# hitmaxiang/pytorch-openpose

Hardware: AMD Instinct MI355X
Metric: frames/sec (body+PAF grouping) at 368x656 (higher is better)
Workload: dtype f32

## Files before the change

### include/opose.h

```cpp
#ifndef OPOSE_H
#define OPOSE_H

#include <stddef.h>
#include <stdint.h>

#ifdef __cplusplus
extern "C" {
#endif

typedef struct opose_ctx opose_t;

typedef enum opose_status {
    OPOSE_OK = 0,
    OPOSE_E_ARG = -1,
    OPOSE_E_SHAPE = -2,
    OPOSE_E_HIP = -3,
    OPOSE_E_WEIGHTS = -4,
    OPOSE_E_CAPACITY = -5,
    OPOSE_E_ASSEMBLY = -6,
    OPOSE_E_TIMEOUT = -7,
} opose_status;

enum { OPOSE_NET_BODY = 0, OPOSE_NET_HAND = 1 };

// ... 124 lines not shown

int opose_profile_enable(opose_t* h, int enable);
int opose_profile_reset(opose_t* h);
int opose_profile_read(opose_t* h, char* buf, size_t len);

int opose_debug_conv(opose_t* h, const float* x, const float* w, const float* b, int N, int Cin, int H, int W,
                     int Cout, int ks, int pad, int relu, int mt, int pt, int splits, float* out);
int opose_debug_conv_time(opose_t* h, int N, int Cin, int H, int W, int Cout, int ks, int ngroups,
                          int mt, int pt, int splits, int ablate, int reps, float* ms);
int opose_debug_conv_x6(opose_t* h, const float* x, const float* w, const float* b, int N, int Cin, int H,
                        int W, int Cout, int ks, int pad, int relu, int mt, int pt, int splits, int out_x6,
                        float* out);
int opose_debug_conv_segs(opose_t* h, int nseg, const int* geom, const float* const* x, int nw,
                          const float* const* w, const float* const* b, int Cin, int Cout, int ks, int relu,
                          int family, int pool, int in_padded, int out_kind, int out_total, int dup, int net,
                          int lvl, int pair, float* const* out, float* const* out_dup, int* ran,
                          int64_t* clobbered);
int opose_debug_chain(opose_t* h, int nseg, const int* geom, const float* const* x, int nw,
                      const float* const* w1, const float* const* b1, const float* const* w2,
                      const float* const* b2, int m1, int cout2, int relu2, int in_padded, int out_x6,
                      float* const* out);
int opose_debug_conv1(opose_t* h, int stage, int nseg, const int* geom, const float* const* x, const float* w,
                      const float* b, int f32, float* const* out);
int opose_debug_conv_x6_time(opose_t* h, int N, int Cin, int H, int W, int Cout, int ks, int ngroups,
                             int mt, int pt, int splits, int reps, float* ms);
int opose_debug_preprocess(opose_t* h, const uint8_t* bgr, int H, int W, double scale, int pad_value,
                           float* out, int* HpWp);
int opose_debug_preprocess_groups(opose_t* h, int n_groups, const uint8_t* const* bgr, const int* N,
                                  const int* H, const int* W, double scale, int pad_value,
                                  float* const* out, int* HpWp);
int opose_debug_heat(opose_t* h, const float* maps, int hl, int wl, int pad_down, int pad_right, int H, int W,
                     double* heat_avg, float* paf_mid);
int opose_debug_hand_label(opose_t* h, const double* maps, int NP, int H, int W, double thre, int32_t* labels,
                           double* sums);
int opose_debug_batch_preprocess(opose_t* h, const uint8_t* bgr, int N, int H, int W, int64_t row_stride,
                                 int64_t frame_stride, double boxsize, double scale, float* out, int* HpWp);
int opose_debug_batch_heat(opose_t* h, const float* maps, int N, int hl, int wl, int nh, int nw, int H, int W,
                           float* heat, float* mid);
int opose_debug_blur5_nms(opose_t* h, const float* heat, int NP, int H, int W, double thre, int cap, int32_t* cnt,
                          int32_t* list, double* score);
int opose_debug_batch_hand_label(opose_t* h, const float* heat, int NP, int H, int W, double thre, double* blurred,
                                 int32_t* labels, double* sums);
int opose_debug_peaks_finalize(opose_t* h, const int32_t* cnt, const int32_t* list, const double* score, int N,
                               int H, int W, void* records, int32_t* peak_pos, int32_t* part_cnt);
int opose_debug_paf_score(opose_t* h, int fast, int n_scales, const float* const* maps, const int* hl, const int* wl,
                          const int* ga, const int* gb, const int32_t* peak_pos, const int32_t* part_cnt, int N,
// ... 18 lines not shown
```

### pytorch-openpose_amd/csrc/conv_win.hip

```cpp
#include <algorithm>
#include <stdexcept>

#include "common.h"
#include "kernels.h"
#include "x6_loop.h"

namespace opose {

template <int MT, int PT, int KS, int WMAX, int NST>
__global__ __launch_bounds__(64 * x6_waves(MT, PT), 1) void conv_win_x6(X6Args a) {
    constexpr int TAPS = KS * KS, PAD = KS / 2;
    constexpr int NW = x6_waves(MT, PT), NWM = NW == 8 ? MT / 64 : 2, NWP = NW / NWM;
    constexpr int WM = MT / NWM, WP = PT / NWP;
    constexpr int TM = WM / 16, TN = WP / 16;
    constexpr int A_U = 12 * MT;
    constexpr int A_PW = A_U / 64 / NW;
    constexpr int WBUF = 3 * WMAX;
    static_assert(A_U % (64 * NW) == 0 && A_PW == 3 && WMAX % 64 == 0 && TAPS >= 9, "conv_win_x6 tile");
    static_assert(NST == 2 || NST == 3, "conv_win_x6 stages");
    constexpr int WOFF = NST * A_U;
    static_assert(TM * TN >= 3, "block 4 hosts the offset steps");

    __shared__ __attribute__((aligned(16))) uint4 lds[NST * A_U + 2 * WBUF];
    __shared__ float s_bias[MT];
// ... 24 lines not shown
        const int n = p / HW, y = (p - n * HW) / W;
        return 3 + n * (H + 3) + y;
    };
    const int p_last = min(p0 + PT, npix) - 1;
    const int R0 = prow(p0), R1 = prow(p_last);
    const int ws = (R0 - PAD) * P;
    const int L = (R1 - R0 + 2 * PAD + 1) * P + PAD;
    const int NQ = (L + 63) >> 6;
    const uint32_t plane0 = G.in_l.o0 - 3u * (uint32_t)P - 3u;
    const int cin_g = a.cin_g;

    auto dma_win = [&](int g) __attribute__((always_inline)) {
        const uint32_t src = (plane0 + (uint32_t)g * G.in_l.gs + (uint32_t)ws) * 16u;
        uint4* dst = lds + WOFF + (g & 1) * WBUF;
        for (int i = wave; i < 3 * NQ; i += NW) {
            const int pc = i / NQ, j = i - pc * NQ;
            const __amdgpu_buffer_rsrc_t rsrc = __builtin_amdgcn_make_buffer_rsrc(
                (void*)(G.in + (size_t)pc * G.in_ps), (short)0, (int)G.in_ps, 0x00020000);
            __builtin_amdgcn_raw_ptr_buffer_load_lds(rsrc, (lds_ptr_t)(dst + pc * WMAX + 64 * j), 16,
                                                     src + (uint32_t)(64 * j + lane) * 16u, 0, 0, 0);
        }
    };
    const uint32_t lane16 = (uint32_t)lane * 16u;
    auto dma_a_unit = [&](int c, int buf, int u) __attribute__((always_inline)) {
        const int unit0 = (wave * A_PW + u) * 64;
        const int pg = unit0 / MT, m = unit0 - pg * MT;
        x6_dma_weights_unit(x6_weights_rsrc(G.wt, a.Mpad, c), (lds_units_t)(lds + buf * A_U), unit0, lane16,
                            (uint32_t)(pg * a.Mpad + m0 + m) * 16u);
    };
    auto dma_a = [&](int c, int buf) __attribute__((always_inline)) {
#pragma unroll
        for (int u = 0; u < A_PW; ++u) dma_a_unit(c, buf, u);
    };

    const int gi = lane >> 4;
    uint32_t bbase[TN];
#pragma unroll
    for (int j = 0; j < TN; ++j) {
        const int p = min(p0 + wp0 + 16 * j + (lane & 15), npix - 1);
        const int n = p / HW, r = p - n * HW, y = r / W, x = r - y * W;
        const int wpos = (3 + n * (H + 3) + y) * P + 3 + x - ws;
        bbase[j] = (uint32_t)(uintptr_t)(lds_ptr_t)(lds + WOFF + wpos);
    }
    int pg_g = (4 * c_begin + gi) / TAPS, pg_t = (4 * c_begin + gi) % TAPS;
    int s_dy = 0, s_dx = 0;
    uint32_t off_n = 0;
    constexpr int OFF_STEPS = 3;
    auto off_step = [&](int k) __attribute__((always_inline)) {
        if (k == 0) {
            s_dy = pg_t / KS;
            s_dx = pg_t - s_dy * KS - PAD;
            s_dy -= PAD;
        } else if (k == 1) {
            off_n = (uint32_t)((min(pg_g, cin_g - 1) & 1) * WBUF * 16 + (s_dy * P + s_dx) * 16);
        } else {
            const int w = pg_t + 4 >= TAPS ? 1 : 0;
            pg_t = pg_t + 4 - w * TAPS;
            pg_g += w;
        }
    };
    auto off_all = [&]() __attribute__((always_inline)) {
#pragma unroll
        for (int k = 0; k < OFF_STEPS; ++k) off_step(k);
    };

    X6Frags<MT, TM, TN> f;
    f.zero();
    constexpr int NB = f.NB, TMN = f.TMN;
    const int a16 = (lane >> 4) * MT + wm0 + (lane & 15);
    auto la = [&](int buf) __attribute__((always_inline)) {
        return (uint32_t)(uintptr_t)(lds_ptr_t)(lds + buf * A_U + a16);
    };

    const int g_first = (4 * c_begin) / TAPS;
    dma_win(g_first);
    if (g_first + 1 < cin_g) dma_win(g_first + 1);
#pragma unroll
    for (int st = 0; st < NST; ++st) dma_a(min(c_begin + st, c_end - 1), st);
    asm volatile("s_waitcnt vmcnt(0)" ::: "memory");
    __syncthreads();
    X6BWin<TN, WMAX> bcur, bnxt;
    {
        off_all();
#pragma unroll
        for (int j = 0; j < TN; ++j) bnxt.a[j] = bbase[j] + off_n;
        off_all();
        f.rd_group(0, la(0), bnxt);
        f.rd_group(1, la(0), bnxt);
    }
    int end_g = g_first;
    int end_c = (g_first * TAPS + TAPS - 1) / 4;
    int buf = 0;
    for (int c = c_begin; c < c_end; ++c) {
        const int nbuf = buf + 1 == NST ? 0 : buf + 1;
        const uint32_t a_cur = la(buf), a_nxt = la(nbuf);
        const int c2 = min(c + NST, c_end - 1);
#pragma unroll
        for (int j = 0; j < TN; ++j) bcur.a[j] = bnxt.a[j];
#pragma unroll
        for (int j = 0; j < TN; ++j) bnxt.a[j] = bbase[j] + off_n;
        f.head(a_cur, bcur);
        f.template barrier<NST == 3 ? A_PW : 0>();
        if (c == end_c) {
            if (end_g + 2 < cin_g) dma_win(end_g + 2);
            ++end_g;
            end_c = (end_g * TAPS + TAPS - 1) / 4;
        }
        __builtin_amdgcn_sched_barrier(0);
#pragma unroll
        for (int q = 0; q < NB; ++q) {
            f.mf(3, q);
            constexpr int N3 = TMN + 1;
#pragma unroll
            for (int o = q * N3 / NB; o < (q + 1) * N3 / NB; ++o) {
                if (o < TMN) f.rd(0, o, a_nxt, bnxt);
                else dma_a_unit(c2, buf, 0);
            }
            __builtin_amdgcn_sched_barrier(0);
        }
#pragma unroll
        for (int q = 0; q < NB; ++q) {
            f.mf(4, q);
            constexpr int N4 = A_PW - 2;
#pragma unroll
            for (int o = q * N4 / NB; o < (q + 1) * N4 / NB; ++o) dma_a_unit(c2, buf, 1 + o);
            if (q < OFF_STEPS) off_step(q);
            __builtin_amdgcn_sched_barrier(0);
        }
#pragma unroll
        for (int q = 0; q < NB; ++q) {
            f.mf(5, q);
            constexpr int N5 = TMN + 1;
#pragma unroll
            for (int o = q * N5 / NB; o < (q + 1) * N5 / NB; ++o) {
                if (o < TMN) f.rd(1, o, a_nxt, bnxt);
                else dma_a_unit(c2, buf, A_PW - 1);
            }
            __builtin_amdgcn_sched_barrier(0);
        }
        buf = nbuf;
    }
    asm volatile("s_waitcnt vmcnt(0) lgkmcnt(0)" ::: "memory");
    f.fence_all();

    if (!un.whole) {
        const __amdgpu_buffer_rsrc_t srs = slab_rsrc(a.partial);
        const uint32_t sbase = (uint32_t)uid * (uint32_t)(MT * PT * 4);
#pragma unroll
        for (int j = 0; j < TN; ++j) {
            const int pl = wp0 + j * 16 + (lane & 15);
#pragma unroll
            for (int i = 0; i < TM; ++i) {
                const int q = (wm0 + i * 16) / 4 + (lane >> 4);
                store_slab_quad(srs, sbase + (uint32_t)(q * PT + pl) * 16u, f.acc[i][j]);
            }
        }
        continue;
    }
    const X6Out out = x6_out(G);
// ... 73 lines not shown
```

### pytorch-openpose_amd/csrc/conv_x6.hip

```cpp
#include <algorithm>
#include <cstdlib>
#include <stdexcept>

#include "common.h"
#include "kernels.h"
#include "x6_loop.h"

namespace opose {

template <int MT, int PT, bool SMALL, int KS>
__global__ __launch_bounds__(64 * x6_waves(MT, PT), 1) void conv_x6(X6Args a) {
    const int ks = KS ? KS : a.ks;
    const int taps = ks * ks;
    constexpr int NW = x6_waves(MT, PT), NWM = NW == 8 ? MT / 64 : 2, NWP = NW / NWM;
    constexpr int WM = MT / NWM, WP = PT / NWP;
    constexpr int TM = WM / 16, TN = WP / 16;
    constexpr int PJ = PT / 64;
    constexpr int A_U = 12 * MT, B_U = 12 * PT;
    constexpr int A_PW = A_U / 64 / NW;
    constexpr int WPJ = NW / PJ;
    constexpr int B_PW = 12 / WPJ;
    static_assert(NW % PJ == 0 && 12 % WPJ == 0 && A_U % (64 * NW) == 0, "x6 tile");

    constexpr int STAGE_U = A_U + B_U;
    __shared__ __attribute__((aligned(16))) uint4 lds[2 * STAGE_U];
// ... 150 lines not shown
            auto mf = [&](int t, int q) __attribute__((always_inline)) {
                const int i = q / TN, j = q % TN;
                acc[i][j] = mfma_x6(fa[kPieceA[t]][i], fb[kPieceB[t]][j], acc[i][j]);
            };
            auto fence_all = [&]() __attribute__((always_inline)) {
#pragma unroll
                for (int pc = 0; pc < 3; ++pc) {
#pragma unroll
                    for (int i = 0; i < TM; ++i) asm volatile("" : "+v"(fa[pc][i]));
#pragma unroll
                    for (int j = 0; j < TN; ++j) asm volatile("" : "+v"(fb[pc][j]));
                }
            };
            dma_a(c_begin, 0);
            dma_b(c_begin, 0);
            asm volatile("s_waitcnt vmcnt(0)" ::: "memory");
            __syncthreads();
            {
                const uint32_t a0 = la(0), b0 = lb(0);
#pragma unroll
                for (int r = 0; r < TMN; ++r) rd(0, r, a0, b0);
#pragma unroll
                for (int r = 0; r < TMN; ++r) rd(1, r, a0, b0);
                const int cn = min(c_begin + 1, c_end - 1);
                dma_a(cn, 1);
                dma_b(cn, 1);
            }
            for (int c = c_begin; c < c_end; ++c) {
                const int buf = (c - c_begin) & 1;
                const uint32_t a_cur = la(buf), b_cur = lb(buf);
                const uint32_t a_nxt = la(buf ^ 1), b_nxt = lb(buf ^ 1);
                const int c2 = min(c + 2, c_end - 1);
                const BPrep bp2 = b_prep(c2);
                asm volatile("s_waitcnt lgkmcnt(%0)" ::"i"(TMN > 15 ? 15 : TMN) : "memory");
                fence_all();
                __builtin_amdgcn_sched_barrier(0);
#pragma unroll
                for (int q = 0; q < NB; ++q) {
                    mf(0, q);
#pragma unroll
                    for (int r = q * TMN / NB; r < (q + 1) * TMN / NB; ++r) rd(2, r, a_cur, b_cur);
                    __builtin_amdgcn_sched_barrier(0);
                }
                asm volatile("s_waitcnt lgkmcnt(%0)" ::"i"(TMN > 15 ? 15 : TMN) : "memory");
                fence_all();
                __builtin_amdgcn_sched_barrier(0);
#pragma unroll
                for (int q = 0; q < NB; ++q) {
                    mf(1, q);
                    __builtin_amdgcn_sched_barrier(0);
                }
                asm volatile("s_waitcnt lgkmcnt(0)" ::: "memory");
                fence_all();
                __builtin_amdgcn_sched_barrier(0);
#pragma unroll
                for (int q = 0; q < NB; ++q) {
                    mf(2, q);
                    __builtin_amdgcn_sched_barrier(0);
                }
                asm volatile("s_waitcnt vmcnt(0)" ::: "memory");
                __syncthreads();
                __builtin_amdgcn_sched_barrier(0);
                constexpr int D3 = NDA / 3, D4 = 2 * NDA / 3;
                auto dma_op = [&](int d) __attribute__((always_inline)) {
                    if (d < A_PW) dma_a_unit(c2, buf, d);
                    else dma_b_unit(c2, bp2, buf, d - A_PW);
                };
#pragma unroll
                for (int q = 0; q < NB; ++q) {
                    mf(3, q);
                    constexpr int N3 = TMN + D3;
#pragma unroll
                    for (int o = q * N3 / NB; o < (q + 1) * N3 / NB; ++o) {
                        if (o < TMN) rd(0, o, a_nxt, b_nxt);
                        else dma_op(o - TMN);
                    }
                    __builtin_amdgcn_sched_barrier(0);
                }
#pragma unroll
                for (int q = 0; q < NB; ++q) {
                    mf(4, q);
                    constexpr int N4 = D4 - D3;
#pragma unroll
                    for (int o = q * N4 / NB; o < (q + 1) * N4 / NB; ++o) dma_op(D3 + o);
                    __builtin_amdgcn_sched_barrier(0);
                }
#pragma unroll
                for (int q = 0; q < NB; ++q) {
                    mf(5, q);
                    constexpr int N5 = TMN + NDA - D4;
#pragma unroll
                    for (int o = q * N5 / NB; o < (q + 1) * N5 / NB; ++o) {
                        if (o < TMN) rd(1, o, a_nxt, b_nxt);
                        else dma_op(D4 + o - TMN);
                    }
                    __builtin_amdgcn_sched_barrier(0);
                }
            }
            asm volatile("s_waitcnt lgkmcnt(0)" ::: "memory");
            fence_all();
        }

        const bool whole = un.whole;
        const X6Out out = x6_out(G);
        const int cout8 = out.cout8;
#pragma unroll
        for (int j = 0; j < TN; ++j) {
            const int pl = wp0 + j * 16 + (lane & 15);
            const int p = p0 + pl;
            auto quad_row = [&](int i) __attribute__((always_inline)) { return wm0 + i * 16 + 4 * (lane >> 4); };
            if (!whole) {
                const __amdgpu_buffer_rsrc_t srs = slab_rsrc(a.partial);
                const uint32_t sbase = (uint32_t)uid * (uint32_t)(MT * PT * 4);
#pragma unroll
                for (int i = 0; i < TM; ++i)
                    store_slab_quad(srs, sbase + (uint32_t)((quad_row(i) / 4) * PT + pl) * 16u, acc[i][j]);
                continue;
            }
            if (a.pool) {
                const int q = p >> 2;
                const int n = q / HWo;
// ... 698 lines not shown
```

### pytorch-openpose_amd/csrc/engine_debug.cpp

```cpp
#include "engine.h"

using namespace opose;

int opose_debug_conv(opose_t* h, const float* x, const float* w, const float* b, int N, int Cin, int H, int W,
                     int Cout, int ks, int pad, int relu, int mt, int pt, int splits, float* out) {
    if (!h || !x || !w || !b || !out || ks > 15 || pad > 7) return OPOSE_E_ARG;
    OPOSE_TRY(h, {
        enter_main(h);
        Spec s{"debug", Cin, Cout, ks, pad};
        upload_conv(h, 0, "__debug__", {&s}, {w}, {b}, 3, false);
        DevConv* c = h->convs[0]["__debug__"].get();
        DevBuf xin, yout;
        const size_t nx = (size_t)N * Cin * H * W, ny = (size_t)N * Cout * H * W;
        float* xd = xin.ensure<float>(nx, h->stream);
        float* yd = yout.ensure<float>(ny, h->stream);
        OPOSE_HIP_CHECK(hipMemcpyAsync(xd, x, nx * 4, hipMemcpyHostToDevice, h->stream));
        ConvArgs a{};
        a.N = N; a.H = H; a.W = W; a.Cin = Cin; a.ks = ks; a.pad = pad;
        a.K = c->K; a.Kpad = c->Kpad; a.Mpad = c->Mpad; a.npix = N * H * W;
        a.tap_major = c->tap_major ? 1 : 0;
        ConvGroup& G = a.g[0];
        G.in = xd; G.in_cstride = Cin; G.in_coff = 0; G.wt = c->wt; G.bias = c->bias;
        G.out = yd; G.out_cstride = Cout; G.out_coff = 0; G.out2 = nullptr; G.cout = Cout; G.relu = relu;
        a.g[1] = a.g[0];
// ... 109 lines not shown
        const uint32_t ips = (uint32_t)((size_t)N * cg * HW * 16), ops = (uint32_t)((size_t)N * og * HW * 16);
        float* xd = xin.ensure<float>(nx, h->stream);
        uint8_t* x6 = xx.ensure<uint8_t>((size_t)ips * 3, h->stream);
        uint8_t* y6 = yx.ensure<uint8_t>((size_t)ops * 3, h->stream);
        float* yd = yout.ensure<float>(ny, h->stream);
        OPOSE_HIP_CHECK(hipMemcpyAsync(xd, x, nx * 4, hipMemcpyHostToDevice, h->stream));
        launch_to_x6(xd, Cin, 0, Cin, N, HW, x6, cg, 0, ips, h->stream);
        X6Args a{};
        a.ks = ks; a.pad = pad;
        a.cin_g = cg; a.small = c->small6 ? 1 : 0; a.nK = c->nK6; a.Mpad = c->Mpad;
        X6Group& G = a.g[0];
        G.N = N; G.H = H; G.W = W; G.npix = N * HW;
        G.in = x6; G.in_ps = ips; G.in_l = x6act(x6, cg, 0, N, H, W).l;
        G.wt = c->wx6; G.bias = c->bias; G.cout = Cout; G.relu = relu; G.out2 = nullptr;
        if (out_x6) { G.out = y6; G.out_ps = ops; G.out_l = x6act(y6, og, 0, N, H, W).l; G.out_f32 = 0; }
        else { G.out = yd; G.out_c = Cout; G.out_off = 0; G.out_f32 = 1; }
        a.ngroups = 1;
        const TileChoice t = debug_x6_plan(h, a, mt, pt, splits);
        launch_conv_x6(a, t.mt, t.pt, h->stream);
        if (out_x6) launch_from_x6(y6, og, 0, ops, Cout, N, HW, yd, Cout, 0, h->stream);
        OPOSE_HIP_CHECK(hipMemcpyAsync(out, yd, ny * 4, hipMemcpyDeviceToHost, h->stream));
        OPOSE_HIP_CHECK(hipStreamSynchronize(h->stream));
        h->convs[0].erase("__debug__");
    });
    return OPOSE_OK;
}

struct DebugConvs {
    opose_ctx* h;
    int net;
    std::vector<std::string> keys;
    DevConv* add(const std::string& key, const Spec& s, const float* w, const float* b, int lvl, bool pair) {
        upload_conv(h, net, key, {&s}, {w}, {b}, lvl, pair);
        keys.push_back(key);
        return h->convs[net][key].get();
    }
    ~DebugConvs() {
        for (const std::string& k : keys) h->convs[net].erase(k);
    }
};

constexpr int kDebugFill = 0xa5;

static int64_t clobbered_units(const uint16_t* hy, const XAct& a, int og, int N, int H, int W) {
    const size_t units = a.ps / 16;
    std::vector<uint8_t> written(units, 0);
// ... 846 lines not shown
```

### pytorch-openpose_amd/csrc/engine_net.cpp

```cpp
#include "engine.h"

namespace opose {

static const NetTable& net_table(opose_ctx* h, int net) {
    if (!h->loaded[net]) throw std::runtime_error(std::string(net_desc(net).what) + " weights not loaded");
    return h->table[net];
}

static void record_gate(opose_ctx* h) {
    if (!h->gate_ev) return;
    OPOSE_HIP_CHECK(hipEventRecord(h->gate_ev, h->stream));
    h->gate_done = true;
}

static const char* conv_class(int ks) { return ks == 7 ? "conv7x7" : (ks == 3 ? "conv3x3" : "conv1x1"); }

static void run_conv(opose_ctx* h, DevConv* c0, DevConv* c1, int N, int H, int W, Act in0, Act out0, Act in1,
                     Act out1, bool relu0, bool relu1, Act dup = {nullptr, 0, 0}) {
    ConvArgs a{};
    const int ng = c1 ? 2 : 1;
    a.N = N;
    a.H = H;
    a.W = W;
    a.Cin = c0->cin;
// ... 118 lines not shown
static XAct frame_view(const XAct& a, int n, int H, int W) {
    XAct v = a;
    if (!a.p) return v;
    if (a.f32) v.p = static_cast<float*>(a.p) + (size_t)n * a.c * H * W;
    else v.l.o0 = a.l.o0 + (uint32_t)n * a.l.fs;
    return v;
}

static std::string layer_names(const std::vector<ConvSeg>& segs) {
    std::string nm = segs[0].c->name;
    for (size_t g = 1; g < segs.size(); ++g)
        if (segs[g].c != segs[0].c && nm.find(segs[g].c->name) == std::string::npos) nm += "|" + segs[g].c->name;
    return "layer/" + nm;
}

static void launch_segs(opose_ctx* h, const std::vector<ConvSeg>& segs, int family, bool pool) {
    const bool win = family == kKernelWin, wino = family == kKernelWino;
    DevConv* c0 = segs[0].c;
    X6Args a{};
    const int ng = (int)segs.size();
    a.ks = c0->ks;
    a.pad = c0->pad;
    a.cin_g = c0->cin_g;
    a.small = c0->small6 ? 1 : 0;
    a.nK = wino ? c0->nKw : win ? c0->nK6p : c0->nK6;
    a.Mpad = c0->Mpad;
    a.pool = pool ? 1 : 0;
    a.ngroups = ng;
    double flops = 0;
    long npix_all = 0;
    for (int g = 0; g < ng; ++g) {
        const ConvSeg& sg = segs[g];
        DevConv* c = sg.c;
        if (c->ks != c0->ks || c->cin_g != c0->cin_g || c->Mpad != c0->Mpad || c->nK6 != c0->nK6 || c->nK6p != c0->nK6p)
            throw std::invalid_argument("conv segments of different shapes");
        if (pool && (sg.dup.p || sg.out.f32)) throw std::invalid_argument("pooled conv: single X6 output only");
        X6Group& G = a.g[g];
        G.in = static_cast<const uint8_t*>(sg.in.p);
        G.in_ps = sg.in.ps;
        G.in_l = sg.in.l;
        G.wt = wino ? c->wwino : win ? c->wx6p : c->wx6;
        G.bias = c->bias;
        G.out = sg.out.p;
        G.out_ps = sg.out.ps;
        G.out_l = sg.out.l;
        G.out_c = sg.out.c;
        G.out_off = sg.out.off;
// ... 538 lines not shown
```

### pytorch-openpose_amd/csrc/engine_plan.cpp

```cpp
#include "engine.h"

namespace opose {

TileChoice choose_tile(int Mpad, const std::vector<int>& gpix, int nK, bool x6, bool dp_only, double* cost_out) {
    long npix_all = 0;
    for (int n : gpix) npix_all += n;
    static const int cfg[6][3] = {{128, 128, 2}, {128, 256, 1}, {256, 128, 1},
                                  {128, 64, 3},  {64, 128, 3},  {64, 64, 4}};
    static const int occ6[6] = {1, 1, 1, 2, 2, 3};
    static const double ovh6_big[6] = {1.5, 1.0, 0.96, 1.1, 1.1, 1.2};
    static const double ovh6_small[6] = {1.0, 1.0, 0.96, 1.1, 1.1, 1.6};
    const double* ovh6 = npix_all <= 16384 ? ovh6_small : ovh6_big;
    const double rate = x6 ? 0.4 : 1.0;
    static const double ovh[6] = {1.0, 0.95, 0.93, 1.02, 1.02, 1.06};
    TileChoice best{64, 64, 1};
    double best_cost = 1e300;
    for (int c = 0; c < 6; ++c) {
        const int mt = cfg[c][0], pt = cfg[c][1], occ = x6 ? occ6[c] : cfg[c][2];
        if (Mpad % mt) continue;
        long tiles = 0;
        for (int n : gpix) tiles += (long)(Mpad / mt) * ((n + pt - 1) / pt);
        const double unit = (mt / 64.0) * (pt / 64.0) * (x6 ? ovh6[c] : ovh[c]) * rate;
        const long per_cu = (tiles + 255) / 256;
        const double floor1 = occ >= 2 ? 1.6 : 1.0;
// ... 149 lines not shown
                          : 0;
    const std::string key = std::to_string(win) + "/" + std::to_string(nK) + "/" + std::to_string(c->Mpad) + "/" +
                            std::to_string(npix) + "/" + std::to_string(mult) + "/" + std::to_string(bpix);
    auto it = h->slab_cache.find(key);
    if (it != h->slab_cache.end()) return it->second;
    static const int cand[] = {1, 2, 3, 4, 5, 6, 7, 8, 10, 12, 14, 16, 20, 24, 28, 32, 40, 48, 64};
    int best = 1;
    double best_cost = 1e300;
    for (int S : cand) {
        if (S > std::max(1, smax)) break;
        double cost = pick_tile(std::vector<ColGroup>(mult, ColGroup{npix, S}), win, nK, c->Mpad).cost;
        if (bpix) cost += pick_tile(std::vector<ColGroup>(mult, ColGroup{bpix, S}), win, nK, c->Mpad, false, false).cost;
        if (cost < best_cost * 0.97) {
            best_cost = cost;
            best = S;
        }
    }
    h->slab_cache[key] = best;
    return best;
}

static int seg_kernel_direct(const opose_ctx* h, const ConvSeg& sg, bool pool) {
    const DevConv* c = sg.c;
    if (!h->win7 || pool || !c->wx6p || !sg.in.padded || (c->ks != 3 && c->ks != 7)) return kKernelX6;
    const long lpix = (long)sg.N * (sg.Hl ? sg.Hl : sg.H) * sg.W;
    if (c->net == OPOSE_NET_BODY && lpix < 4096) return kKernelX6;
    if (c->net == OPOSE_NET_HAND && c->ks == 3 && c->lvl == 3 && c->Mpad > 128) return kKernelX6;
    if (sg.N == 1) return conv_win_fits_rows(sg.W, c->ks) ? kKernelWin : kKernelX6;
    if (conv_win_fits(sg.N, sg.H, sg.W, c->ks)) return kKernelWin;
    if (c->ks == 7 && h->split_frames && conv_win_fits_rows(sg.W, c->ks)) return kKernelWinFrames;
    return kKernelX6;
}

int seg_kernel(opose_ctx* h, const ConvSeg& sg, bool pool) {
    if (h->force_kernel >= 0) return h->force_kernel;
    const int k = seg_kernel_direct(h, sg, pool);
    const DevConv* c = sg.c;
    if (k == kKernelWin && h->wino && c->ks == 3 && c->wwino &&
        slab_count(h, c, true, sg.N, sg.Hl ? sg.Hl : sg.H, sg.W, pool) == 1 &&
        wino_tpf(sg.N, sg.Hl ? sg.Hl : sg.H, sg.W) >= 0)
        return kKernelWino;
    return k;
}

ConvPlan plan_launch(opose_ctx* h, const std::vector<ConvSeg>& segs, bool win, bool pool, int nK, int Mpad) {
    std::string key = (win ? "w" : "x") + std::to_string(pool) + "/" + std::to_string(nK) + "/" + std::to_string(Mpad);
    for (const ConvSeg& s : segs)
// ... 39 lines not shown
```

### pytorch-openpose_amd/csrc/engine_weights.cpp

```cpp
#include "engine.h"

namespace opose {

static DevConv* find_conv(opose_ctx* h, int net, const std::string& name) {
    auto it = h->convs[net].find(name);
    if (it == h->convs[net].end()) throw std::runtime_error("missing layer " + name);
    return it->second.get();
}

void upload_conv(opose_ctx* h, int net, const std::string& key, const std::vector<const Spec*>& parts,
                 const std::vector<const float*>& w, const std::vector<const float*>& b, int lvl, bool pair,
                 const std::vector<int>& cmap) {
    auto dc = std::make_unique<DevConv>();
    const Spec& s0 = *parts[0];
    dc->name = key;
    dc->net = net;
    dc->lvl = lvl;
    dc->pair = pair;
    dc->cin = s0.cin;
    dc->ks = s0.ks;
    dc->pad = s0.pad;
    dc->K = s0.cin * s0.ks * s0.ks;
    dc->tap_major = s0.cin >= 32;
    const int cin_pad = round_up(s0.cin, 32);
// ... 18 lines not shown
    std::vector<int> ktab(dc->Kpad, 0);
    for (int k = 0; k < dc->K; ++k) {
        int c = k / (dc->ks * dc->ks), r = k % (dc->ks * dc->ks);
        ktab[k] = (c << 8) | ((r / dc->ks) << 4) | (r % dc->ks);
    }
    {
        const int cin_phys = cmap.empty() ? s0.cin : cmap.back() + 1;
        const int taps = s0.ks * s0.ks;
        std::vector<float> wp((size_t)cout * cin_phys * taps, 0.f);
        int mm = 0;
        for (size_t i = 0; i < parts.size(); ++i)
            for (int m = 0; m < parts[i]->cout; ++m, ++mm)
                for (int c = 0; c < s0.cin; ++c) {
                    const int pc = cmap.empty() ? c : cmap[c];
                    for (int t = 0; t < taps; ++t)
                        wp[((size_t)mm * cin_phys + pc) * taps + t] = w[i][((size_t)m * s0.cin + c) * taps + t];
                }
        std::vector<uint16_t> wx;
        x6_pack_weights(wp.data(), cout, cin_phys, s0.ks, dc->Mpad, &dc->nK6, wx);
        dc->cin_g = (cin_phys + 7) / 8;
        dc->small6 = dc->cin_g == 1;
        OPOSE_HIP_CHECK(hipMalloc(&dc->wx6, wx.size() * 2));
        OPOSE_HIP_CHECK(hipMemcpy(dc->wx6, wx.data(), wx.size() * 2, hipMemcpyHostToDevice));
        if ((s0.ks == 7 || s0.ks == 3) && dc->Mpad % 128 == 0 && cin_phys > 8) {
            x6_pack_weights_pairs(wp.data(), cout, cin_phys, s0.ks, dc->Mpad, &dc->nK6p, wx);
            OPOSE_HIP_CHECK(hipMalloc(&dc->wx6p, wx.size() * 2));
            OPOSE_HIP_CHECK(hipMemcpy(dc->wx6p, wx.data(), wx.size() * 2, hipMemcpyHostToDevice));
        }
        if (s0.ks == 3 && dc->Mpad % 128 == 0 && cin_phys > 8) {
            x6_pack_weights_wino(wp.data(), cout, cin_phys, dc->Mpad, &dc->nKw, wx);
            OPOSE_HIP_CHECK(hipMalloc(&dc->wwino, wx.size() * 2));
            OPOSE_HIP_CHECK(hipMemcpy(dc->wwino, wx.data(), wx.size() * 2, hipMemcpyHostToDevice));
        }
    }
    OPOSE_HIP_CHECK(hipMalloc(&dc->wt, wt.size() * 4));
    OPOSE_HIP_CHECK(hipMalloc(&dc->bias, bias.size() * 4));
    OPOSE_HIP_CHECK(hipMalloc(&dc->ktab, ktab.size() * 4));
    g_alloc_epoch.fetch_add(1);
    OPOSE_HIP_CHECK(hipMemcpy(dc->wt, wt.data(), wt.size() * 4, hipMemcpyHostToDevice));
    OPOSE_HIP_CHECK(hipMemcpy(dc->bias, bias.data(), bias.size() * 4, hipMemcpyHostToDevice));
    OPOSE_HIP_CHECK(hipMemcpy(dc->ktab, ktab.data(), ktab.size() * 4, hipMemcpyHostToDevice));
    h->convs[net][key] = std::move(dc);
}

}

using namespace opose;
// ... 50 lines not shown
```

### pytorch-openpose_amd/csrc/x6.h

```cpp
#pragma once
#include <hip/hip_runtime.h>

#include "common.h"

namespace opose {

typedef float f32x4 __attribute__((ext_vector_type(4)));
typedef __bf16 bf16x8 __attribute__((ext_vector_type(8)));
typedef int i32x4 __attribute__((ext_vector_type(4)));
typedef __attribute__((address_space(3))) void* lds_ptr_t;
typedef __attribute__((address_space(3))) uint4* lds_units_t;

namespace x6 {

constexpr int x6_waves(int mt, int pt) { return mt * pt >= 32768 ? 8 : 4; }

__device__ __forceinline__ uint32_t bf16_rne(float x) {
    uint32_t u = __float_as_uint(x);
    u += 0x7fffu + ((u >> 16) & 1u);
    return u >> 16;
}

__device__ __forceinline__ void split3(float x, uint32_t& h0, uint32_t& h1, uint32_t& h2) {
    h0 = bf16_rne(x);
    const float r = x - __uint_as_float(h0 << 16);
    h1 = bf16_rne(r);
    const float r2 = r - __uint_as_float(h1 << 16);
    h2 = bf16_rne(r2);
}

__device__ __forceinline__ float join3(uint32_t h0, uint32_t h1, uint32_t h2) {
    return (__uint_as_float(h0 << 16) + __uint_as_float(h1 << 16)) + __uint_as_float(h2 << 16);
}

__device__ __forceinline__ void pack_pieces4(const float (&v)[4], uint2 (&w)[3]) {
    uint32_t h[3][4];
#pragma unroll
    for (int t = 0; t < 4; ++t) split3(v[t], h[0][t], h[1][t], h[2][t]);
#pragma unroll
    for (int pc = 0; pc < 3; ++pc) {
        w[pc].x = h[pc][0] | (h[pc][1] << 16);
        w[pc].y = h[pc][2] | (h[pc][3] << 16);
    }
}
__device__ __forceinline__ void pack_pieces8(const float (&v)[8], uint4 (&w)[3]) {
    uint32_t h[3][8];
#pragma unroll
    for (int t = 0; t < 8; ++t) split3(v[t], h[0][t], h[1][t], h[2][t]);
#pragma unroll
    for (int pc = 0; pc < 3; ++pc) {
        w[pc].x = h[pc][0] | (h[pc][1] << 16);
        w[pc].y = h[pc][2] | (h[pc][3] << 16);
        w[pc].z = h[pc][4] | (h[pc][5] << 16);
        w[pc].w = h[pc][6] | (h[pc][7] << 16);
    }
}
__device__ __forceinline__ void store4_x6(uint8_t* unit, uint32_t ps, const float (&v)[4]) {
    uint2 w[3];
    pack_pieces4(v, w);
#pragma unroll
    for (int pc = 0; pc < 3; ++pc) *reinterpret_cast<uint2*>(unit + (size_t)pc * ps) = w[pc];
}
__device__ __forceinline__ void store8_x6(uint8_t* unit, uint32_t ps, const float (&v)[8]) {
    uint4 w[3];
    pack_pieces8(v, w);
#pragma unroll
    for (int pc = 0; pc < 3; ++pc) *reinterpret_cast<uint4*>(unit + (size_t)pc * ps) = w[pc];
}

constexpr int kPieceA[6] = {0, 0, 0, 1, 2, 1};
constexpr int kPieceB[6] = {2, 0, 1, 0, 0, 1};
__device__ __forceinline__ f32x4 mfma_x6(const i32x4& a, const i32x4& b, f32x4 c) {
    return __builtin_amdgcn_mfma_f32_16x16x32_bf16(__builtin_bit_cast(bf16x8, a), __builtin_bit_cast(bf16x8, b), c, 0,
                                                   0, 0);
}

__device__ __forceinline__ int x6_xcd_id() { return xcd_contiguous_id(gridDim.x, blockIdx.x); }

__device__ __forceinline__ void x6_load_bias(float* s_bias, const X6Group& G, int m0, int MT) {
    const int tid = threadIdx.x;
    if (tid < MT) s_bias[tid] = (m0 + tid < G.cout) ? G.bias[m0 + tid] : 0.f;
}

__device__ __forceinline__ void x6_dma_weights_unit(__amdgpu_buffer_rsrc_t rsrc, lds_units_t stage, int unit0,
                                                    uint32_t lane16, uint32_t soffset) {
    __builtin_amdgcn_raw_ptr_buffer_load_lds(rsrc, (lds_ptr_t)(stage + unit0), 16, lane16, (int)soffset, 0, 0);
}
__device__ __forceinline__ __amdgpu_buffer_rsrc_t x6_weights_rsrc(const uint8_t* wt, int Mpad, int c) {
    return __builtin_amdgcn_make_buffer_rsrc((void*)(wt + (size_t)c * 12 * Mpad * 16), (short)0, (int)0x7fffffff,
                                             0x00020000);
}

__device__ __forceinline__ __amdgpu_buffer_rsrc_t slab_rsrc(float* partial) {
    return __builtin_amdgcn_make_buffer_rsrc((void*)partial, (short)0, 0x7fffffff, 0x00020000);
}
__device__ __forceinline__ void store_slab_quad(__amdgpu_buffer_rsrc_t r, uint32_t byte_off, f32x4 v) {
    typedef unsigned u32x4 __attribute__((ext_vector_type(4)));
    __builtin_amdgcn_raw_buffer_store_b128(__builtin_bit_cast(u32x4, v), r, (int)byte_off, 0, 16);
}

__device__ __forceinline__ uint32_t x6_unit(const X6Layout& l, int n, int g, int y, int x) {
    return l.o0 + (uint32_t)n * l.fs + (uint32_t)g * l.gs + (uint32_t)y * l.rs + (uint32_t)x;
}

struct X6Out {
    void *out, *out2;
    uint32_t out_ps, out2_ps;
    X6Layout out_l, out2_l;
    int out_c, out_off, cout, cout8, out_f32;
};
__device__ __forceinline__ X6Out x6_out(const X6Group& G) {
    return X6Out{G.out,   G.out2,    G.out_ps, G.out2_ps,        G.out_l, G.out2_l,
                 G.out_c, G.out_off, G.cout,   (G.cout + 7) & ~7, G.out_f32};
// ... 58 lines not shown
```

### pytorch-openpose_amd/csrc/x6_loop.h

```cpp
#pragma once
#include "x6.h"

namespace opose {
namespace x6 {

template <int TN, int WMAX>
struct X6BWin {
    uint32_t a[TN];
    __device__ __forceinline__ uint32_t addr(int j) const { return a[j]; }
    static constexpr int off(int pc, int) { return pc * WMAX * 16; }
};

template <int MT, int TM, int TN>
struct X6Frags {
    static constexpr int NB = TM * TN;
    static constexpr int TMN = TM + TN;
    i32x4 fa[3][TM], fb[3][TN];
    f32x4 acc[TM][TN];

    __device__ __forceinline__ void zero() {
#pragma unroll
        for (int i = 0; i < TM; ++i)
#pragma unroll
            for (int j = 0; j < TN; ++j) acc[i][j] = f32x4{0.f, 0.f, 0.f, 0.f};
// ... 39 lines not shown
            for (int r = q * TMN / NB; r < (q + 1) * TMN / NB; ++r) rd(2, r, a_cur, b_cur);
            __builtin_amdgcn_sched_barrier(0);
        }
        asm volatile("s_waitcnt lgkmcnt(%0)" ::"i"(TMN > 15 ? 15 : TMN) : "memory");
        fence_all();
        __builtin_amdgcn_sched_barrier(0);
#pragma unroll
        for (int q = 0; q < NB; ++q) {
            mf(1, q);
            __builtin_amdgcn_sched_barrier(0);
        }
        asm volatile("s_waitcnt lgkmcnt(0)" ::: "memory");
        fence_all();
        __builtin_amdgcn_sched_barrier(0);
#pragma unroll
        for (int q = 0; q < NB; ++q) {
            mf(2, q);
            __builtin_amdgcn_sched_barrier(0);
        }
    }
    template <int VMCNT>
    __device__ __forceinline__ void barrier() {
        asm volatile("s_waitcnt vmcnt(%0)" ::"i"(VMCNT) : "memory");
        __syncthreads();
        __builtin_amdgcn_sched_barrier(0);
    }
};

}
}
```

### pytorch-openpose_amd/src/_native.py

```python
from __future__ import annotations

import ctypes as C
import os

import numpy as np

_HERE = os.path.dirname(os.path.abspath(__file__))
LIB_PATH = os.environ.get("OPOSE_LIB", os.path.join(os.path.dirname(_HERE), "lib", "libopose.so"))

OPOSE_OK = 0
OPOSE_E_ARG, OPOSE_E_SHAPE, OPOSE_E_HIP, OPOSE_E_WEIGHTS, OPOSE_E_CAPACITY, OPOSE_E_ASSEMBLY = -1, -2, -3, -4, -5, -6
OPOSE_E_TIMEOUT = -7
NET_BODY, NET_HAND = 0, 1
IN_DEVICE, OUT_DEVICE, PIPELINE, PIPELINE_DEFER = 1, 2, 4, 8
DEVICE_IO = IN_DEVICE | OUT_DEVICE
MAX_SCALES = 8


class Params(C.Structure):
    _fields_ = [("n_scales", C.c_int), ("scales", C.c_double * MAX_SCALES), ("boxsize", C.c_double),
                ("stride", C.c_int), ("pad_value", C.c_int), ("thre1", C.c_double), ("thre2", C.c_double),
                ("thre_hand", C.c_double)]


# ... 36 lines not shown
    "opose_hand_post": (_I, [_P, C.POINTER(_P), _P, _P, _P, _P, _I, _I, _I, _I, C.POINTER(Params), _P, _P, _I]),
    "opose_hand_infer_crops": (_I, [_P, C.POINTER(_P), _P, _P, _I, C.POINTER(Params), _P, _P, _I]),
    "opose_batch_body_infer": (_I, [_P, _P, _I, _I, _I, _L, _L, C.POINTER(Params), _P, _I]),
    "opose_batch_body_post": (_I, [_P, _P, _I, _I, _I, _I, _I, _I, _I, C.POINTER(Params), _P, _I]),
    "opose_batch_hand_infer": (_I, [_P, _P, _I, _I, _I, _L, _L, C.POINTER(Params), _P, _P, _I]),
    "opose_batch_hand_post": (_I, [_P, _P, _I, _I, _I, C.POINTER(Params), _P, _P, _I]),
    "opose_batch_hand_boxes": (_I, [_P, _P, _I, _I, _I, _P, _I]),
    "opose_batch_hand_crops": (_I, [_P, _P, _I, _I, _I, _L, _L, _P, _I, _P, _I]),
    "opose_batch_hand_extract": (_I, [_P, _P, _I, _I, _I, _L, _L, _P, _I, C.POINTER(Params), _P, _P, _I]),
    "opose_body_records_pose": (_I, [_P, _P, _I, _P, _P, _I]),
    "opose_batch_body_extract": (_I, [_P, _P, _I, _I, _I, _L, _L, C.POINTER(Params), _P, _P, _I]),
    "opose_profile_enable": (_I, [_P, _I]),
    "opose_profile_reset": (_I, [_P]),
    "opose_profile_read": (_I, [_P, C.c_char_p, _S]),
    "opose_debug_conv": (_I, [_P, _P, _P, _P, _I, _I, _I, _I, _I, _I, _I, _I, _I, _I, _I, _P]),
    "opose_debug_preprocess": (_I, [_P, _P, _I, _I, _D, _I, _P, _P]),
    "opose_debug_preprocess_groups": (_I, [_P, _I, C.POINTER(_P), _P, _P, _P, _D, _I, C.POINTER(_P), _P]),
    "opose_debug_conv_time": (_I, [_P, _I, _I, _I, _I, _I, _I, _I, _I, _I, _I, _I, _I, _P]),
    "opose_debug_conv_x6": (_I, [_P, _P, _P, _P, _I, _I, _I, _I, _I, _I, _I, _I, _I, _I, _I, _I, _P]),
    "opose_debug_conv_segs": (_I, [_P, _I, _P, _P, _I, _P, _P, _I, _I, _I, _I, _I, _I, _I, _I, _I, _I, _I, _I, _I, _P, _P, _P,
                                   _P]),
    "opose_debug_chain": (_I, [_P, _I, _P, _P, _I, _P, _P, _P, _P, _I, _I, _I, _I, _I, _P]),
    "opose_debug_conv1": (_I, [_P, _I, _I, _P, _P, _P, _P, _I, _P]),
    "opose_debug_conv_x6_time": (_I, [_P, _I, _I, _I, _I, _I, _I, _I, _I, _I, _I, _I, _P]),
    "opose_debug_heat": (_I, [_P, _P, _I, _I, _I, _I, _I, _I, _P, _P]),
    "opose_debug_hand_label": (_I, [_P, _P, _I, _I, _I, _D, _P, _P]),
    "opose_debug_batch_preprocess": (_I, [_P, _P, _I, _I, _I, _L, _L, _D, _D, _P, _P]),
    "opose_debug_batch_heat": (_I, [_P, _P, _I, _I, _I, _I, _I, _I, _I, _P, _P]),
    "opose_debug_blur5_nms": (_I, [_P, _P, _I, _I, _I, _D, _I, _P, _P, _P]),
    "opose_debug_batch_hand_label": (_I, [_P, _P, _I, _I, _I, _D, _P, _P, _P]),
    "opose_debug_peaks_finalize": (_I, [_P, _P, _P, _P, _I, _I, _I, _P, _P, _P]),
    "opose_debug_paf_score": (_I, [_P, _I, _I, _P, _P, _P, _P, _P, _P, _P, _I, _I, _I, _D, _P]),
    "opose_debug_limb_greedy": (_I, [_P, _P, _P, _I, _P, _P, _P, _P]),
    "opose_debug_assemble": (_I, [_P, _P, _P, _P, _P, _P, _P, _I, _P]),
    "opose_debug_hand_crops": (_I, [_P, _P, _I, _I, _I, _L, _L, _P, _I, _P, _P, _P]),
    "opose_debug_hand_backmap": (_I, [_P, _P, _P, _P, _I, _I, _P]),
    "opose_draw_records": (_I, [_P, _P, _I, _I, _I, _L, _L, _P, _P, _P, _I]),
    "opose_draw_motion": (_I, [_P, _P, _I, _I, _I, _L, _L, _P, _I, _P, _P, _I]),
    "opose_debug_draw_prims": (_I, [_P, _P, _I, _I, _I, _I, _P, _P, _P]),
}
EXPORTED = list(SIGNATURES)


def _load():
    if not os.path.exists(LIB_PATH):
        raise ImportError(f"libopose.so not found at {LIB_PATH}: build it with `make -C pytorch-openpose_amd` "
# ... 239 lines not shown
```

Baseline: 2143.

## Trim redundant tail prefetches, use packed bf16 converts, widen windowed-kernel eligibility

The windowed and x6 conv kernels stop issuing redundant weight and window DMAs past the last chunk. Dead weight loads get a zero-size buffer resource, and the x6 loop gets a separate tail-chunk instantiation that skips prefetch. The fp32-to-3xbf16 split now uses a packed two-value vector convert, and the loop barrier drops __syncthreads for a bare s_barrier. Eligibility for the windowed kernel and pair-packed weights is widened to cin_phys==8 while excluding cin_g<2, and a debug entry point for the split is added. The risks are changed kernel selection for some layers and subtle synchronization or rounding differences.

```diff
diff --git a/include/opose.h b/include/opose.h
--- a/include/opose.h
+++ b/include/opose.h
@@ -170,6 +170,7 @@
                       float* const* out);
 int opose_debug_conv1(opose_t* h, int stage, int nseg, const int* geom, const float* const* x, const float* w,
                       const float* b, int f32, float* const* out);
+int opose_debug_split_pieces(opose_t* h, const float* x, int64_t n, uint16_t* pieces);
 int opose_debug_conv_x6_time(opose_t* h, int N, int Cin, int H, int W, int Cout, int ks, int ngroups,
                              int mt, int pt, int splits, int reps, float* ms);
 int opose_debug_preprocess(opose_t* h, const uint8_t* bgr, int H, int W, double scale, int pad_value,
diff --git a/pytorch-openpose_amd/csrc/conv_win.hip b/pytorch-openpose_amd/csrc/conv_win.hip
--- a/pytorch-openpose_amd/csrc/conv_win.hip
+++ b/pytorch-openpose_amd/csrc/conv_win.hip
@@ -70,15 +70,15 @@
         }
     };
     const uint32_t lane16 = (uint32_t)lane * 16u;
-    auto dma_a_unit = [&](int c, int buf, int u) __attribute__((always_inline)) {
+    auto dma_a_unit = [&](int c, int buf, int u, bool live) __attribute__((always_inline)) {
         const int unit0 = (wave * A_PW + u) * 64;
         const int pg = unit0 / MT, m = unit0 - pg * MT;
-        x6_dma_weights_unit(x6_weights_rsrc(G.wt, a.Mpad, c), (lds_units_t)(lds + buf * A_U), unit0, lane16,
+        x6_dma_weights_unit(x6_weights_rsrc(G.wt, a.Mpad, c, live), (lds_units_t)(lds + buf * A_U), unit0, lane16,
                             (uint32_t)(pg * a.Mpad + m0 + m) * 16u);
     };
-    auto dma_a = [&](int c, int buf) __attribute__((always_inline)) {
-#pragma unroll
-        for (int u = 0; u < A_PW; ++u) dma_a_unit(c, buf, u);
+    auto dma_a = [&](int c, int buf, bool live) __attribute__((always_inline)) {
+#pragma unroll
+        for (int u = 0; u < A_PW; ++u) dma_a_unit(c, buf, u, live);
     };
 
     const int gi = lane >> 4;
@@ -121,12 +121,18 @@
     };
 
     const int g_first = (4 * c_begin) / TAPS;
+    const int g_last = min((4 * c_end - 1) / TAPS, cin_g - 1);
+    const bool win2 = g_first < g_last;
+    const bool win2_now = win2 && (4 * c_begin + 3) / TAPS > g_first;
     dma_win(g_first);
-    if (g_first + 1 < cin_g) dma_win(g_first + 1);
-#pragma unroll
-    for (int st = 0; st < NST; ++st) dma_a(min(c_begin + st, c_end - 1), st);
+    if (win2_now) dma_win(g_first + 1);
+    dma_a(c_begin, 0, true);
     asm volatile("s_waitcnt vmcnt(0)" ::: "memory");
     __syncthreads();
+    dma_a(min(c_begin + 1, c_end - 1), 1, c_begin + 1 < c_end);
+    if (win2 && !win2_now) dma_win(g_first + 1);
+    if (NST == 3) dma_a(min(c_begin + 2, c_end - 1), 2, c_begin + 2 < c_end);
+    __builtin_amdgcn_sched_barrier(0);
     X6BWin<TN, WMAX> bcur, bnxt;
     {
         off_all();
@@ -143,6 +149,7 @@
         const int nbuf = buf + 1 == NST ? 0 : buf + 1;
         const uint32_t a_cur = la(buf), a_nxt = la(nbuf);
         const int c2 = min(c + NST, c_end - 1);
+        const bool live = c + NST < c_end;
 #pragma unroll
         for (int j = 0; j < TN; ++j) bcur.a[j] = bnxt.a[j];
 #pragma unroll
@@ -150,7 +157,7 @@
         f.head(a_cur, bcur);
         f.template barrier<NST == 3 ? A_PW : 0>();
         if (c == end_c) {
-            if (end_g + 2 < cin_g) dma_win(end_g + 2);
+            if (end_g + 2 <= g_last) dma_win(end_g + 2);
             ++end_g;
             end_c = (end_g * TAPS + TAPS - 1) / 4;
         }
@@ -162,7 +169,7 @@
 #pragma unroll
             for (int o = q * N3 / NB; o < (q + 1) * N3 / NB; ++o) {
                 if (o < TMN) f.rd(0, o, a_nxt, bnxt);
-                else dma_a_unit(c2, buf, 0);
+                else dma_a_unit(c2, buf, 0, live);
             }
             __builtin_amdgcn_sched_barrier(0);
         }
@@ -171,7 +178,7 @@
             f.mf(4, q);
             constexpr int N4 = A_PW - 2;
 #pragma unroll
-            for (int o = q * N4 / NB; o < (q + 1) * N4 / NB; ++o) dma_a_unit(c2, buf, 1 + o);
+            for (int o = q * N4 / NB; o < (q + 1) * N4 / NB; ++o) dma_a_unit(c2, buf, 1 + o, live);
             if (q < OFF_STEPS) off_step(q);
             __builtin_amdgcn_sched_barrier(0);
         }
@@ -182,7 +189,7 @@
 #pragma unroll
             for (int o = q * N5 / NB; o < (q + 1) * N5 / NB; ++o) {
                 if (o < TMN) f.rd(1, o, a_nxt, bnxt);
-                else dma_a_unit(c2, buf, A_PW - 1);
+                else dma_a_unit(c2, buf, A_PW - 1, live);
             }
             __builtin_amdgcn_sched_barrier(0);
         }
diff --git a/pytorch-openpose_amd/csrc/conv_x6.hip b/pytorch-openpose_amd/csrc/conv_x6.hip
--- a/pytorch-openpose_amd/csrc/conv_x6.hip
+++ b/pytorch-openpose_amd/csrc/conv_x6.hip
@@ -1,6 +1,7 @@
 #include <algorithm>
 #include <cstdlib>
 #include <stdexcept>
+#include <type_traits>
 
 #include "common.h"
 #include "kernels.h"
@@ -197,16 +198,18 @@
                 for (int r = 0; r < TMN; ++r) rd(0, r, a0, b0);
 #pragma unroll
                 for (int r = 0; r < TMN; ++r) rd(1, r, a0, b0);
-                const int cn = min(c_begin + 1, c_end - 1);
-                dma_a(cn, 1);
-                dma_b(cn, 1);
-            }
-            for (int c = c_begin; c < c_end; ++c) {
+                if (c_begin + 1 < c_end) {
+                    dma_a(c_begin + 1, 1);
+                    dma_b(c_begin + 1, 1);
+                }
+            }
+            auto chunk = [&](int c, auto tail) __attribute__((always_inline)) {
+                constexpr bool TAIL = decltype(tail)::value;
                 const int buf = (c - c_begin) & 1;
                 const uint32_t a_cur = la(buf), b_cur = lb(buf);
                 const uint32_t a_nxt = la(buf ^ 1), b_nxt = lb(buf ^ 1);
-                const int c2 = min(c + 2, c_end - 1);
-                const BPrep bp2 = b_prep(c2);
+                const int c2 = c + 2;
+                const BPrep bp2 = TAIL ? BPrep{0u, 0} : b_prep(c2);
                 asm volatile("s_waitcnt lgkmcnt(%0)" ::"i"(TMN > 15 ? 15 : TMN) : "memory");
                 fence_all();
                 __builtin_amdgcn_sched_barrier(0);
@@ -238,6 +241,7 @@
                 __builtin_amdgcn_sched_barrier(0);
                 constexpr int D3 = NDA / 3, D4 = 2 * NDA / 3;
                 auto dma_op = [&](int d) __attribute__((always_inline)) {
+                    if (TAIL) return;
                     if (d < A_PW) dma_a_unit(c2, buf, d);
                     else dma_b_unit(c2, bp2, buf, d - A_PW);
                 };
@@ -271,7 +275,10 @@
                     }
                     __builtin_amdgcn_sched_barrier(0);
                 }
-            }
+            };
+            int c = c_begin;
+            for (; c < c_end - 2; ++c) chunk(c, std::false_type{});
+            for (; c < c_end; ++c) chunk(c, std::true_type{});
             asm volatile("s_waitcnt lgkmcnt(0)" ::: "memory");
             fence_all();
         }
diff --git a/pytorch-openpose_amd/csrc/engine_debug.cpp b/pytorch-openpose_amd/csrc/engine_debug.cpp
--- a/pytorch-openpose_amd/csrc/engine_debug.cpp
+++ b/pytorch-openpose_amd/csrc/engine_debug.cpp
@@ -155,6 +155,28 @@
         OPOSE_HIP_CHECK(hipMemcpyAsync(out, yd, ny * 4, hipMemcpyDeviceToHost, h->stream));
         OPOSE_HIP_CHECK(hipStreamSynchronize(h->stream));
         h->convs[0].erase("__debug__");
+    });
+    return OPOSE_OK;
+}
+
+int opose_debug_split_pieces(opose_t* h, const float* x, int64_t n, uint16_t* pieces) {
+    if (!h || !x || !pieces || n < 8 || n % 8 || n > (1 << 24)) return OPOSE_E_ARG;
+    OPOSE_TRY(h, {
+        enter_main(h);
+        const int HW = (int)(n / 8);
+        const uint32_t ps = (uint32_t)HW * 16u;
+        DevBuf xin, xx;
+        float* xd = xin.ensure<float>((size_t)n, h->stream);
+        uint8_t* x6 = xx.ensure<uint8_t>((size_t)ps * 3, h->stream);
+        OPOSE_HIP_CHECK(hipMemcpyAsync(xd, x, (size_t)n * 4, hipMemcpyHostToDevice, h->stream));
+        launch_to_x6(xd, 8, 0, 8, 1, HW, x6, 1, 0, ps, h->stream);
+        std::vector<uint16_t> hy((size_t)3 * n);
+        OPOSE_HIP_CHECK(hipMemcpyAsync(hy.data(), x6, (size_t)ps * 3, hipMemcpyDeviceToHost, h->stream));
+        OPOSE_HIP_CHECK(hipStreamSynchronize(h->stream));
+        for (int pc = 0; pc < 3; ++pc)
+            for (int c = 0; c < 8; ++c)
+                for (int p = 0; p < HW; ++p)
+                    pieces[(size_t)pc * n + (size_t)c * HW + p] = hy[(size_t)pc * n + (size_t)p * 8 + c];
     });
     return OPOSE_OK;
 }
diff --git a/pytorch-openpose_amd/csrc/engine_net.cpp b/pytorch-openpose_amd/csrc/engine_net.cpp
--- a/pytorch-openpose_amd/csrc/engine_net.cpp
+++ b/pytorch-openpose_amd/csrc/engine_net.cpp
@@ -164,7 +164,7 @@
     a.ks = c0->ks;
     a.pad = c0->pad;
     a.cin_g = c0->cin_g;
-    a.small = c0->small6 ? 1 : 0;
+    a.small = c0->small6 && !win && !wino ? 1 : 0;
     a.nK = wino ? c0->nKw : win ? c0->nK6p : c0->nK6;
     a.Mpad = c0->Mpad;
     a.pool = pool ? 1 : 0;
diff --git a/pytorch-openpose_amd/csrc/engine_plan.cpp b/pytorch-openpose_amd/csrc/engine_plan.cpp
--- a/pytorch-openpose_amd/csrc/engine_plan.cpp
+++ b/pytorch-openpose_amd/csrc/engine_plan.cpp
@@ -195,7 +195,7 @@
 
 static int seg_kernel_direct(const opose_ctx* h, const ConvSeg& sg, bool pool) {
     const DevConv* c = sg.c;
-    if (!h->win7 || pool || !c->wx6p || !sg.in.padded || (c->ks != 3 && c->ks != 7)) return kKernelX6;
+    if (!h->win7 || pool || !c->wx6p || c->cin_g < 2 || !sg.in.padded || (c->ks != 3 && c->ks != 7)) return kKernelX6;
     const long lpix = (long)sg.N * (sg.Hl ? sg.Hl : sg.H) * sg.W;
     if (c->net == OPOSE_NET_BODY && lpix < 4096) return kKernelX6;
     if (c->net == OPOSE_NET_HAND && c->ks == 3 && c->lvl == 3 && c->Mpad > 128) return kKernelX6;
diff --git a/pytorch-openpose_amd/csrc/engine_weights.cpp b/pytorch-openpose_amd/csrc/engine_weights.cpp
--- a/pytorch-openpose_amd/csrc/engine_weights.cpp
+++ b/pytorch-openpose_amd/csrc/engine_weights.cpp
@@ -64,7 +64,7 @@
         dc->small6 = dc->cin_g == 1;
         OPOSE_HIP_CHECK(hipMalloc(&dc->wx6, wx.size() * 2));
         OPOSE_HIP_CHECK(hipMemcpy(dc->wx6, wx.data(), wx.size() * 2, hipMemcpyHostToDevice));
-        if ((s0.ks == 7 || s0.ks == 3) && dc->Mpad % 128 == 0 && cin_phys > 8) {
+        if ((s0.ks == 7 || s0.ks == 3) && dc->Mpad % 128 == 0 && cin_phys >= 8) {
             x6_pack_weights_pairs(wp.data(), cout, cin_phys, s0.ks, dc->Mpad, &dc->nK6p, wx);
             OPOSE_HIP_CHECK(hipMalloc(&dc->wx6p, wx.size() * 2));
             OPOSE_HIP_CHECK(hipMemcpy(dc->wx6p, wx.data(), wx.size() * 2, hipMemcpyHostToDevice));
diff --git a/pytorch-openpose_amd/csrc/x6.h b/pytorch-openpose_amd/csrc/x6.h
--- a/pytorch-openpose_amd/csrc/x6.h
+++ b/pytorch-openpose_amd/csrc/x6.h
@@ -15,18 +15,18 @@
 
 constexpr int x6_waves(int mt, int pt) { return mt * pt >= 32768 ? 8 : 4; }
 
-__device__ __forceinline__ uint32_t bf16_rne(float x) {
-    uint32_t u = __float_as_uint(x);
-    u += 0x7fffu + ((u >> 16) & 1u);
-    return u >> 16;
+__device__ __forceinline__ uint32_t bf16_rne2(float a, float b) {
+    typedef float f32x2 __attribute__((ext_vector_type(2)));
+    typedef __bf16 bf16x2 __attribute__((ext_vector_type(2)));
+    return __builtin_bit_cast(uint32_t, __builtin_convertvector(f32x2{a, b}, bf16x2));
 }
 
-__device__ __forceinline__ void split3(float x, uint32_t& h0, uint32_t& h1, uint32_t& h2) {
-    h0 = bf16_rne(x);
-    const float r = x - __uint_as_float(h0 << 16);
-    h1 = bf16_rne(r);
-    const float r2 = r - __uint_as_float(h1 << 16);
-    h2 = bf16_rne(r2);
+__device__ __forceinline__ void split3x2(float a, float b, uint32_t& w0, uint32_t& w1, uint32_t& w2) {
+    w0 = bf16_rne2(a, b);
+    const float ra = a - __uint_as_float(w0 << 16), rb = b - __uint_as_float(w0 & 0xffff0000u);
+    w1 = bf16_rne2(ra, rb);
+    const float sa = ra - __uint_as_float(w1 << 16), sb = rb - __uint_as_float(w1 & 0xffff0000u);
+    w2 = bf16_rne2(sa, sb);
 }
 
 __device__ __forceinline__ float join3(uint32_t h0, uint32_t h1, uint32_t h2) {
@@ -34,26 +34,14 @@
 }
 
 __device__ __forceinline__ void pack_pieces4(const float (&v)[4], uint2 (&w)[3]) {
-    uint32_t h[3][4];
-#pragma unroll
-    for (int t = 0; t < 4; ++t) split3(v[t], h[0][t], h[1][t], h[2][t]);
-#pragma unroll
-    for (int pc = 0; pc < 3; ++pc) {
-        w[pc].x = h[pc][0] | (h[pc][1] << 16);
-        w[pc].y = h[pc][2] | (h[pc][3] << 16);
-    }
+    split3x2(v[0], v[1], w[0].x, w[1].x, w[2].x);
+    split3x2(v[2], v[3], w[0].y, w[1].y, w[2].y);
 }
 __device__ __forceinline__ void pack_pieces8(const float (&v)[8], uint4 (&w)[3]) {
-    uint32_t h[3][8];
-#pragma unroll
-    for (int t = 0; t < 8; ++t) split3(v[t], h[0][t], h[1][t], h[2][t]);
-#pragma unroll
-    for (int pc = 0; pc < 3; ++pc) {
-        w[pc].x = h[pc][0] | (h[pc][1] << 16);
-        w[pc].y = h[pc][2] | (h[pc][3] << 16);
-        w[pc].z = h[pc][4] | (h[pc][5] << 16);
-        w[pc].w = h[pc][6] | (h[pc][7] << 16);
-    }
+    split3x2(v[0], v[1], w[0].x, w[1].x, w[2].x);
+    split3x2(v[2], v[3], w[0].y, w[1].y, w[2].y);
+    split3x2(v[4], v[5], w[0].z, w[1].z, w[2].z);
+    split3x2(v[6], v[7], w[0].w, w[1].w, w[2].w);
 }
 __device__ __forceinline__ void store4_x6(uint8_t* unit, uint32_t ps, const float (&v)[4]) {
     uint2 w[3];
@@ -86,9 +74,9 @@
                                                     uint32_t lane16, uint32_t soffset) {
     __builtin_amdgcn_raw_ptr_buffer_load_lds(rsrc, (lds_ptr_t)(stage + unit0), 16, lane16, (int)soffset, 0, 0);
 }
-__device__ __forceinline__ __amdgpu_buffer_rsrc_t x6_weights_rsrc(const uint8_t* wt, int Mpad, int c) {
-    return __builtin_amdgcn_make_buffer_rsrc((void*)(wt + (size_t)c * 12 * Mpad * 16), (short)0, (int)0x7fffffff,
-                                             0x00020000);
+__device__ __forceinline__ __amdgpu_buffer_rsrc_t x6_weights_rsrc(const uint8_t* wt, int Mpad, int c, bool live = true) {
+    return __builtin_amdgcn_make_buffer_rsrc((void*)(wt + (size_t)c * 12 * Mpad * 16), (short)0,
+                                             live ? (int)0x7fffffff : 0, 0x00020000);
 }
 
 __device__ __forceinline__ __amdgpu_buffer_rsrc_t slab_rsrc(float* partial) {
diff --git a/pytorch-openpose_amd/csrc/x6_loop.h b/pytorch-openpose_amd/csrc/x6_loop.h
--- a/pytorch-openpose_amd/csrc/x6_loop.h
+++ b/pytorch-openpose_amd/csrc/x6_loop.h
@@ -85,7 +85,7 @@
     template <int VMCNT>
     __device__ __forceinline__ void barrier() {
         asm volatile("s_waitcnt vmcnt(%0)" ::"i"(VMCNT) : "memory");
-        __syncthreads();
+        __builtin_amdgcn_s_barrier();
         __builtin_amdgcn_sched_barrier(0);
     }
 };
diff --git a/pytorch-openpose_amd/src/_native.py b/pytorch-openpose_amd/src/_native.py
--- a/pytorch-openpose_amd/src/_native.py
+++ b/pytorch-openpose_amd/src/_native.py
@@ -82,6 +82,7 @@
                                    _P]),
     "opose_debug_chain": (_I, [_P, _I, _P, _P, _I, _P, _P, _P, _P, _I, _I, _I, _I, _I, _P]),
     "opose_debug_conv1": (_I, [_P, _I, _I, _P, _P, _P, _P, _I, _P]),
+    "opose_debug_split_pieces": (_I, [_P, _P, _L, _P]),
     "opose_debug_conv_x6_time": (_I, [_P, _I, _I, _I, _I, _I, _I, _I, _I, _I, _I, _I, _P]),
     "opose_debug_heat": (_I, [_P, _P, _I, _I, _I, _I, _I, _I, _P, _P]),
     "opose_debug_hand_label": (_I, [_P, _P, _I, _I, _I, _D, _P, _P]),
```

New measurement: 2159 (median of 6 runs). No clear change (+0.8%).
